# jgkellymit/GENIE-SMEM

Measured on AMD Instinct MI355X. Metric: query-bases/sec SMEM discovery, 100kb ref x 150bp reads; bit-exact SMEM set, higher is better.
Workload: dtype u8/int32 (2-bit packed bases, int32 SA rows; f64 only in the RMI predict)

## Files before the change

genie-smem_amd/csrc/kernels.hip:

```cpp
#include <hip/hip_runtime.h>

#include <algorithm>
#include <cstdio>
#include <cstdlib>
#include <mutex>
#include <string>
#include <unordered_map>

#include "genie_internal.h"

namespace genie {

namespace {

constexpr int kWave = 64;

__device__ __forceinline__ int rfl(int v) { return __builtin_amdgcn_readfirstlane(v); }
__device__ __forceinline__ void set_wave_priority(int i)
{
    switch (i & 3) {
    case 0: __builtin_amdgcn_s_setprio(0); break;
    case 1: __builtin_amdgcn_s_setprio(1); break;
    case 2: __builtin_amdgcn_s_setprio(2); break;
    default: __builtin_amdgcn_s_setprio(3); break;
// ... 455 lines not shown
__device__ __forceinline__ unsigned long long wave_inclusive_scan64(unsigned long long v, int lane)
{
#pragma unroll
    for (int off = 1; off < kWave; off <<= 1) {
        const unsigned int lo = (unsigned)__shfl_up((int)(unsigned)v, off, kWave);
        const unsigned int hi = (unsigned)__shfl_up((int)(unsigned)(v >> 32), off, kWave);
        if (lane >= off) v += ((unsigned long long)hi << 32) | lo;
    }
    return v;
}

__global__ void __launch_bounds__(kScanBlock) compact_block_sums(const int32_t *__restrict__ counts, long long N, int cap,
                                                                 unsigned long long *__restrict__ block_sums)
{
    __shared__ unsigned long long wsum[kScanBlock / kWave];
    const long long i = (long long)blockIdx.x * kScanBlock + threadIdx.x;
    unsigned long long v = 0;
    if (i < N) { const int c = counts[i]; v = (unsigned long long)(c < 0 ? 0 : (c < cap ? c : cap)); }
    v = wave_sum64(v);
    if ((threadIdx.x & 63) == 0) wsum[threadIdx.x >> 6] = v;
    __syncthreads();
    if (threadIdx.x == 0) {
        unsigned long long s = 0;
        for (int w = 0; w < kScanBlock / kWave; w++) s += wsum[w];
        block_sums[blockIdx.x] = s;
    }
}

__global__ void __launch_bounds__(kScanBlock) scan_block_sums_kernel(unsigned long long *__restrict__ sums, long long nblocks)
{
    constexpr int kPer = 8;
    __shared__ unsigned long long wave_total[kScanBlock / kWave];
    __shared__ unsigned long long carry;
    const int lane = threadIdx.x & (kWave - 1), wave = threadIdx.x >> 6;
    if (threadIdx.x == 0) carry = 0;
    __syncthreads();
    for (long long base = 0; base < nblocks; base += (long long)kScanBlock * kPer) {
        const long long i0 = base + (long long)threadIdx.x * kPer;
        unsigned long long v[kPer], mine = 0;
#pragma unroll
        for (int e = 0; e < kPer; e++) {
            v[e] = i0 + e < nblocks ? sums[i0 + e] : 0ull;
            mine += v[e];
        }
        unsigned long long inc = mine;
#pragma unroll
        for (int off = 1; off < kWave; off <<= 1) {
            const unsigned int lo = (unsigned)__shfl_up((int)(unsigned)inc, off, kWave);
            const unsigned int hi = (unsigned)__shfl_up((int)(unsigned)(inc >> 32), off, kWave);
            if (lane >= off) inc += ((unsigned long long)hi << 32) | lo;
        }
        if (lane == kWave - 1) wave_total[wave] = inc;
        __syncthreads();
        unsigned long long before = carry, all = 0;
        for (int w = 0; w < kScanBlock / kWave; w++) {
            const unsigned long long t = wave_total[w];
            before += w < wave ? t : 0ull;
            all += t;
        }
        unsigned long long run = before + inc - mine;
#pragma unroll
        for (int e = 0; e < kPer; e++) {
            if (i0 + e < nblocks) sums[i0 + e] = run;
            run += v[e];
        }
        __syncthreads();
        if (threadIdx.x == 0) carry += all;
        __syncthreads();
    }
    if (threadIdx.x == 0) sums[nblocks] = carry;
}

__global__ void __launch_bounds__(kScanBlock) compact_scatter(const int32_t *__restrict__ counts,
                                                              const int4 *__restrict__ slots, long long N, int cap,
                                                              const unsigned long long *__restrict__ block_sums,
                                                              long long *__restrict__ offsets, int4 *__restrict__ out,
                                                              long long out_cap_rows)
{
    __shared__ unsigned long long wave_total[kScanBlock / kWave];
    const int lane = threadIdx.x & (kWave - 1), wave = threadIdx.x >> 6;
    const long long i = (long long)blockIdx.x * kScanBlock + threadIdx.x;
    unsigned long long v = 0;
    if (i < N) { const int c = counts[i]; v = (unsigned long long)(c < 0 ? 0 : (c < cap ? c : cap)); }
    const unsigned long long inc = wave_inclusive_scan64(v, lane);
    if (lane == kWave - 1) wave_total[wave] = inc;
    __syncthreads();
    unsigned long long base = block_sums[blockIdx.x] + inc - v;
    for (int w = 0; w < wave; w++) base += wave_total[w];
    if (i < N) {
        offsets[i] = (long long)base;
        if (i == N - 1) offsets[N] = (long long)(base + v);
        if (out) {
            const long long room = out_cap_rows - (long long)base;
            const unsigned int fit = room <= 0 ? 0u : (room < (long long)v ? (unsigned int)room : (unsigned int)v);
            for (unsigned int t = 0; t < fit; t++) out[base + t] = slots[i * (long long)cap + t];
        }
    }
}

std::mutex g_err_mu;
std::string g_err;

#define HIP_TRY(expr)                                                         \
    do {                                                                      \
        hipError_t e_ = (expr);                                               \
        if (e_ != hipSuccess) { set_hip_error(#expr, (int)e_); return GENIE_E_HIP; } \
    } while (0)

#define LAUNCH(kernel, grid, block, lds, stream, ...)                         \
    do {                                                                      \
        hipLaunchKernelGGL(kernel, grid, block, lds, stream, __VA_ARGS__);    \
        HIP_TRY(hipGetLastError());                                           \
    } while (0)

inline long long table_bytes(const genie_index *ix)
{
    return (long long)((ix->dev.flags & kFlagCompactTable) ? sizeof(MatchRec16) : sizeof(MatchRec)) * ix->dev.mtab_entries;
}

struct Geometry {
    int grid, block, lds;
    int grp;
    int wps;
    int wide;
    int max_len;
    int fwd_stride;
    int fwd_lds;
    int qp_recs;
    int qp_stride;
    int kj_row;
};

inline void shape_for(int max_len, Geometry *g)
{
    g->max_len = max_len;
    g->wide = max_len > 255;
    g->qp_recs = g->wide ? (max_len + 31) / 32 : ((max_len + 8 + 31) / 32 + 1 + 1) / 2;
    g->fwd_stride = g->wide ? ((max_len * 2) + 15) & ~15 : std::max(16, (max_len + 15) & ~15);
    int dw = std::max(1, (max_len + 3) / 4);
    if ((dw & 1) == 0) dw++;
    g->fwd_lds = dw * 4;
    g->kj_row = (std::max(max_len, 1) + 1 + 7) & ~7;
    g->qp_stride = g->wide ? g->qp_recs : g->qp_recs + kPairHeadWords * 8 / 16;
}

int plan_find_smems(const genie_index *ix, int mode, int max_len, long long N, Geometry *g)
{
    (void)mode;
    const int lds_cap = 160 * 1024;
    shape_for(max_len, g);
    const int cus = ix->num_cus > 0 ? ix->num_cus : 256;
    const int wpb = 8;
    long long per_block;
    if (g->wide) {
        g->grp = 1;
        g->lds = wpb * mt_long_wave_bytes(max_len, g->qp_recs) + 16;
        per_block = wpb;
    } else {
        const int ml = std::max(max_len, 1);
        const int grp = ix->opt_group_positions > 0 ? ix->opt_group_positions / ml : kMtTarget / ml;
        g->grp = std::max(1, std::min(std::min(kMtMaxG, kWave / mt_pack_dwords(ml) * 4), grp));
        g->lds = wpb * mt_wave_bytes(g->grp, ml, g->qp_recs, g->fwd_stride) + 16 + mt_quad_table_bytes(g->grp, ml);
        per_block = (long long)wpb * g->grp;
    }
    if (g->lds > lds_cap) return GENIE_E_TOO_LONG;
    g->block = wpb * kWave;
    g->wps = !g->wide && table_bytes(ix) > kTableFitsL2 ? 4 : ((ix->dev.flags & kFlagCompactTable) ? 6 : 8);
    int bpc = std::min(lds_cap / g->lds, 4 * g->wps / wpb);
    if (ix->opt_search_blocks_per_cu > 0) bpc = std::min(bpc, ix->opt_search_blocks_per_cu);
    if (bpc < 1) bpc = 1;
    long long gr = (long long)cus * bpc;
    const long long need = (N + per_block - 1) / per_block;
    if (gr > need) gr = need;
    if (gr < 1) gr = 1;
    g->grid = (int)gr;
    return GENIE_OK;
}

struct Workspace {
    uint8_t *fwd;
    RefRec *qp;
    int32_t *status;
    uint8_t *kj;
    int32_t *counts;
    uint8_t *scan_tmp;
    int32_t *vlens;
};

inline int64_t ws_align(int64_t x) { return (x + 255) & ~(int64_t)255; }

struct Carver {
    uint8_t *base;
    int64_t at = 0;
    template <class T> void take(T *&piece, int64_t bytes)
    {
        piece = base ? reinterpret_cast<T *>(base + at) : nullptr;
        at += ws_align(bytes);
    }
};

template <class F>
inline long long pass_size(long long lo, long long total, F fits)
{
    long long hi = std::max(lo, total);
    while (lo < hi) {
        const long long mid = lo + (hi - lo + 1) / 2;
        if (fits(mid)) lo = mid; else hi = mid - 1;
    }
    return std::min(lo, total);
}

inline int64_t block_sums_bytes(int64_t N) { return (N / 16 + 3) * 8; }

inline int64_t workspace_layout(uint8_t *base, int64_t N, const Geometry &g, Workspace *ws, int64_t vlens_n = 0)
{
    Carver c{base};
    c.take(ws->fwd, N * (int64_t)g.fwd_stride);
    c.take(ws->qp, N * (int64_t)g.qp_stride * 16);
    c.take(ws->status, N * 4);
    c.take(ws->kj, N * (int64_t)g.kj_row * (g.wide ? 4 : 2));
    c.take(ws->counts, N * 4);
    c.take(ws->scan_tmp, block_sums_bytes(N));
    c.take(ws->vlens, vlens_n * 4);
    return c.at + 256;
}

inline int carve_workspace(void *d_ws, int64_t ws_bytes, int64_t N, const Geometry &g, Workspace *ws, int64_t vlens_n = 0)
{
    if (!d_ws || ws_bytes < workspace_layout(static_cast<uint8_t *>(d_ws), N, g, ws, vlens_n) || (reinterpret_cast<uintptr_t>(d_ws) & 255) != 0)
        return GENIE_E_CAPACITY;
    return GENIE_OK;
}

constexpr long long kLongTwoLaneReads = 32768;

struct FindRequest : FindBatch {
    int32_t *counts = nullptr, *slots = nullptr;
    int32_t cap = 0;
    int64_t *offsets = nullptr;
    int32_t *rows = nullptr;
    int64_t cap_rows = 0;
    bool packed = false;
    int row_bytes = 8;
    uint8_t *counts8 = nullptr, *status8 = nullptr;
    int64_t *escapes = nullptr;
    int64_t cap_escapes = 0;
    bool both = false;

    explicit FindRequest(const FindBatch &b) : FindBatch(b) {}
};

constexpr int kLdsBytes = 160 * 1024;
std::mutex g_lds_mu;
std::unordered_map<const void *, int> g_lds_limit;

template <class Kernel>
int allow_large_lds(Kernel k)
{
    const void *fn = reinterpret_cast<const void *>(k);
    int limit;
    {
        std::lock_guard<std::mutex> lk(g_lds_mu);
        auto it = g_lds_limit.find(fn);
        if (it == g_lds_limit.end()) {
            hipFuncAttributes attr;
            HIP_TRY(hipFuncGetAttributes(&attr, fn));
            it = g_lds_limit.emplace(fn, kLdsBytes - (int)attr.sharedSizeBytes).first;
        }
        limit = it->second;
    }
    HIP_TRY(hipFuncSetAttribute(fn, hipFuncAttributeMaxDynamicSharedMemorySize, limit));
    return GENIE_OK;
}

template <class Kernel, class... Args>
int launch_match_table(Kernel km, const Geometry &g, hipStream_t s, Args... args)
{
    if (int rc = allow_large_lds(km)) return rc;
    LAUNCH(km, dim3(g.grid), dim3(g.block), g.lds, s, args...);
    return GENIE_OK;
}

inline auto pick_interval_rows(bool c16, bool packed, int row_bytes) -> decltype(&interval_rows_kernel<true, 0>)
{
    if (!packed) return c16 ? interval_rows_kernel<true, 0> : interval_rows_kernel<false, 0>;
    if (row_bytes == 6) return c16 ? interval_rows_kernel<true, 2> : interval_rows_kernel<false, 2>;
    return c16 ? interval_rows_kernel<true, 1> : interval_rows_kernel<false, 1>;
}
inline auto pick_interval(bool csr, bool wide, bool c16) -> decltype(&interval_kernel<false, false, true>)
{
    if (csr) return c16 ? interval_kernel<true, true, true> : interval_kernel<true, true, false>;
    if (wide) return c16 ? interval_kernel<false, true, true> : interval_kernel<false, true, false>;
    return c16 ? interval_kernel<false, false, true> : interval_kernel<false, false, false>;
}

template <int MODE, bool WIDE>
int launch_pipeline(const genie_index *ix, const Geometry &g, const FindRequest &r, const Workspace &ws, hipStream_t s)
{
    int32_t *st = r.status ? r.status : ws.status;
    int32_t *cnt = r.counts ? r.counts : ws.counts;
    const bool c16 = (ix->dev.flags & kFlagCompactTable) != 0;
    const long long mtab_bytes = table_bytes(ix);
    const int cus = ix->num_cus > 0 ? ix->num_cus : 256;
    const int max_len = std::max(g.max_len, 1);
    const int long_flags = ix->opt_search_all | ix->opt_scheduling << 16, flags = long_flags | ix->opt_debug << 8;
    if (ix->ev_search_begin) HIP_TRY(hipEventRecord((hipEvent_t)ix->ev_search_begin, s));
    int rc;
    if (WIDE && r.both)
        rc = launch_match_table(c16 ? match_table_long_both_kernel<true> : match_table_long_both_kernel<false>, g, s, ix->dev,
                                (int)MODE, r.reads, r.lens, (long long)r.N, r.stride, r.fixed_len, reinterpret_cast<uint8_t *>(ws.fwd),
                                g.fwd_stride, ws.qp, g.qp_recs, st, max_len, mtab_bytes, long_flags, cus, ws.vlens);
    else if (WIDE)
        rc = launch_match_table(c16 ? match_table_long_kernel<true> : match_table_long_kernel<false>, g, s, ix->dev, (int)MODE,
                                r.reads, r.lens, (long long)r.N, r.stride, r.fixed_len, reinterpret_cast<uint8_t *>(ws.fwd),
                                g.fwd_stride, ws.qp, g.qp_recs, st, max_len, mtab_bytes, long_flags, cus);
    else if (r.both)
        rc = launch_match_table(c16 ? (g.wps == 4 ? match_table_both_kernel<4, true> : match_table_both_kernel<6, true>)
                                    : (g.wps == 4 ? match_table_both_kernel<4, false> : match_table_both_kernel<8, false>),
                                g, s, ix->dev, (int)MODE, r.reads, r.lens, (long long)r.N, r.stride, r.fixed_len,
                                reinterpret_cast<uint8_t *>(ws.fwd), g.fwd_stride, ws.qp, g.qp_recs, g.qp_stride, st, g.grp,
// ... 430 lines not shown
```

genie-smem_amd/csrc/match_table_body.inc:

```
    static_assert(!(PK && RC), "both strands of 2-bit packed reads are not built");
    typedef uint32_t __attribute__((aligned(1))) u32_unaligned;
    extern __shared__ __align__(16) uint8_t smem[];
    const int lane = threadIdx.x & (kWave - 1);
    const int wave = rfl((int)(threadIdx.x >> 6));
    const int waves_per_block = blockDim.x >> 6;
    const int dbg = (flags >> 8) & 63;
    const int sched = flags >> 16;
    const bool look_up_all = (flags & 1) != 0;
    const int FS = fwd_stride;
    const int K = ix.K;
    const int P2 = ix.P2;
    const int DW = mt_short_row_dwords(max_len, qp_recs);
    const int DWp = mt_pack_dwords(max_len);
    const int QL = mt_quads(max_len);
    const int nquads = grp * QL;
    const __amdgpu_buffer_rsrc_t mtab =
        __builtin_amdgcn_make_buffer_rsrc(const_cast<MatchRec *>(ix.mtab), 0, (int)mtab_bytes, 0x00020000);
    const __amdgpu_buffer_rsrc_t ov =
        __builtin_amdgcn_make_buffer_rsrc(const_cast<MatchOv16 *>(ix.ov), 0, ix.ov_entries * (int)sizeof(MatchOv16), 0x00020000);

    uint8_t *wb = smem + wave * mt_wave_bytes(grp, max_len, qp_recs, FS);
    uint32_t *Dp = reinterpret_cast<uint32_t *>(wb);
    int *Ls = reinterpret_cast<int *>(wb + mt_r16(grp * DW * 4));
    uint8_t *fwL = reinterpret_cast<uint8_t *>(Ls) + 64;
    uint16_t *sl = reinterpret_cast<uint16_t *>(fwL + mt_r16(grp * FS));
    uint16_t *qa = reinterpret_cast<uint16_t *>(reinterpret_cast<uint8_t *>(sl) + mt_r16(grp * max_len * 2));
    uint16_t *qb = qa + grp * mt_quads(max_len);
    for (int i = lane; i < grp * DW; i += kWave) Dp[i] = 0;
    const uint8_t *reads_end = reads + (RC ? N >> 1 : N) * (long long)stride;

    const int pu = (int)(((uint32_t)lane * (uint32_t)(65536 / DWp + 1)) >> 16);
    const int pj = lane - pu * DWp;

    uint32_t *next_group = reinterpret_cast<uint32_t *>(smem + waves_per_block * mt_wave_bytes(grp, max_len, qp_recs, FS));
    const long long groups = (N + grp - 1) / grp;
    const long long share = (groups + gridDim.x - 1) / gridDim.x;
    const long long g_begin = (long long)blockIdx.x * share;
    const long long g_end = g_begin + share < groups ? g_begin + share : groups;
    const bool handed_out = !(sched & 1), rotate = !(sched & 2);
    if (threadIdx.x == 0) *next_group = (uint32_t)waves_per_block;
    uint2 *qtab = reinterpret_cast<uint2 *>(next_group + 4);
    for (int t = threadIdx.x; t < (nquads + 191) / 192 * 192; t += blockDim.x) {
        const int tq = t < nquads ? t : 0;
        const int u = tq / QL, a = 4 * (tq - u * QL);
        const uint32_t o = 2u * (uint32_t)a + 1u;
        qtab[t] = make_uint2((uint32_t)u << 28 | (uint32_t)(u * FS + a) << 16 | (uint32_t)a,
                             ((uint32_t)(u * DW) + (o >> 5)) << 8 | (32u - (o & 31u)));
    }
    __syncthreads();
    long long gi = handed_out ? g_begin + wave : (long long)blockIdx.x * waves_per_block + wave;
    const long long g_stop = handed_out ? g_end : groups;
    const int round_of_block = (int)(blockIdx.x / (uint32_t)cus);
    const bool touch_ahead = !(sched & 8);
    for (int it = 0; gi < g_stop; it++) {
        const long long r = gi * grp;
        if (rotate) set_wave_priority(it + round_of_block);
        long long gi_next;
        if (handed_out) {
            uint32_t nx = 0;
            if (lane == 0) nx = atomicAdd(next_group, 1u);
            gi_next = g_begin + (long long)(uint32_t)rfl((int)nx);
        } else {
            gi_next = gi + (long long)gridDim.x * waves_per_block;
        }
        if (touch_ahead && stride > 0 && gi_next < g_stop) {
            const long long rn = gi_next * grp;
            const long long rows = N - rn < (long long)grp ? N - rn : (long long)grp;
            if (RC) scalar_touch_lines(reads + (rn >> 1) * (long long)stride, (uint32_t)((((rn + rows - 1) >> 1) - (rn >> 1) + 1) * stride));
            else scalar_touch_lines(reads + rn * (long long)stride, (uint32_t)(rows * stride));
        }
        bool any_read = false;
        for (int u0 = 0; u0 < grp; u0 += kWave / DWp) {
            const int u = u0 + pu;
            const bool mine = pu < kWave / DWp && u < grp;
            int L = 0, st = GENIE_READ_OK;
            uint32_t d = 0;
            bool bad = false;
            if (mine && r + u < N) {
                const long long row = RC ? (r + u) >> 1 : r + u;
                const bool rev = RC && ((r + u) & 1);
                L = lens ? lens[row] : fixed_len;
                if (RC && lens && pj == 0) vlens[r + u] = L;
                if (L < 0 || L > max_len) { st = GENIE_READ_BAD_BASE; L = 0; }
                const int left = L - 16 * pj;
                if (PK) {
                    if (left > 0) {
                        d = __builtin_bswap32(*reinterpret_cast<const uint32_t *>(reads + (r + u) * (long long)stride + 4 * pj));
                        if (left < 16) d &= ~0u << (32 - 2 * left);
                    }
                }
                const uint8_t *src = reads + row * (long long)stride + 16 * pj;
                uint32_t v[4] = {0, 0, 0, 0};
                if (PK) {
                } else if (rev) {
                    const long long o = row * (long long)stride + L - 16 - 16 * pj;
                    if (left >= 16 || (left > 0 && o >= 0)) {
                        const nt_u4 q = *reinterpret_cast<const nt_u4_unaligned *>(reads + o);
                        v[0] = __builtin_bswap32(q.w); v[1] = __builtin_bswap32(q.z); v[2] = __builtin_bswap32(q.y); v[3] = __builtin_bswap32(q.x);
                        if (left < 16) {
#pragma unroll
                            for (int k = 0; k < 4; k++) {
                                const int nb = left - 4 * k;
                                v[k] = nb >= 4 ? v[k] : (nb <= 0 ? 0u : v[k] & ((1u << (8 * nb)) - 1u));
                            }
                        }
                    } else if (left > 0) {
                        const uint8_t *f = reads + row * (long long)stride;
                        for (int b = 0; b < left; b++) v[b >> 2] |= (uint32_t)f[left - 1 - b] << (8 * (b & 3));
                    }
                } else if (left >= 16 || (left > 0 && src + 16 <= reads_end)) {
                    const nt_u4 q = *reinterpret_cast<const nt_u4_unaligned *>(src);
                    v[0] = q.x; v[1] = q.y; v[2] = q.z; v[3] = q.w;
                    if (left < 16) {
#pragma unroll
                        for (int k = 0; k < 4; k++) {
                            const int nb = left - 4 * k;
                            v[k] = nb >= 4 ? v[k] : (nb <= 0 ? 0u : v[k] & ((1u << (8 * nb)) - 1u));
                        }
                    }
                } else if (left > 0) {
#pragma unroll
                    for (int k = 0; k < 4; k++) {
                        if (left >= 4 * k + 4) v[k] = *reinterpret_cast<const u32_unaligned *>(src + 4 * k);
                        else for (int b = 0; b < left - 4 * k; b++) v[k] |= (uint32_t)src[4 * k + b] << (8 * b);
                    }
                }
                if (!PK) {
                    bad = ((v[0] | v[1] | v[2] | v[3]) & 0xFCFCFCFCu) != 0;
                    d = (mt_pack4(v[0]) << 24) | (mt_pack4(v[1]) << 16) | (mt_pack4(v[2]) << 8) | mt_pack4(v[3]);
                    if (rev && left > 0) d ^= left >= 16 ? ~0u : ~0u << (32 - 2 * left);
                }
            }
            const uint32_t prev = (uint32_t)__builtin_amdgcn_update_dpp(0, (int)d, 0x138 , 0xf, 0xf, true);
            const unsigned long long badm = __ballot(bad);
            bool ok = false;
            if (mine) {
                Dp[u * DW + pj] = __builtin_amdgcn_alignbit(prev, d, 1);
                if (pj == 0) {
                    const unsigned long long mine_bits = ((1ull << DWp) - 1ull) << (pu * DWp);
                    if (st == GENIE_READ_OK && (badm & mine_bits)) st = GENIE_READ_BAD_BASE;
                    if (st == GENIE_READ_OK && mode != GENIE_MODE_BWA && L < K) st = GENIE_READ_TOO_SHORT;
                    if (r + u < N) status[r + u] = st;
                    ok = st == GENIE_READ_OK && L > 0;
                    Ls[u] = ok ? L : 0;
                }
            }
            any_read |= __any(ok);
        }
        wave_lds_fence();
        if (any_read) {
            for (int t0 = 0; t0 < ((dbg & 8) ? 0 : grp * qp_recs); t0 += kWave) {
                const int t = t0 + lane;
                const int u = t / qp_recs, i = t - u * qp_recs;
                if (t < grp * qp_recs && Ls[u] > 0) {
                    const uint32_t *q = Dp + u * DW + 4 * i;
                    const uint32_t q0 = q[0], q1 = q[1], q2 = q[2], q3 = q[3], q4 = q[4];
                    uint4 rec;
                    rec.y = __builtin_amdgcn_alignbit(q0, q1, 31);
                    rec.x = __builtin_amdgcn_alignbit(q1, q2, 31);
                    rec.w = __builtin_amdgcn_alignbit(q2, q3, 31);
                    rec.z = __builtin_amdgcn_alignbit(q3, q4, 31);
                    store_nt(qp_out + (r + u) * (long long)qp_stride + i, rec);
                }
            }
            int nslow = 0;
#pragma nounroll
            for (int c0 = 0; c0 < ((dbg & 4) ? 0 : nquads); c0 += kMtNsp * kWave) {
                uint32_t ent[kMtNsp];
                MtProbe pr[kMtNsp];
#pragma unroll
                for (int s = 0; s < kMtNsp; s++) {
                    const int t0 = c0 + 64 * s + lane;
                    const uint2 q = qtab[t0];
                    int m = Ls[q.x >> 28] - (int)(q.x & 255u);
                    m = t0 < nquads && m > 0 ? m : 0;
                    ent[s] = q.x | ((uint32_t)m << 8);
                    const uint32_t *dq = Dp + (q.y >> 8);
                    const uint32_t sh = q.y & 255u;
                    const uint32_t d0 = dq[0], d1 = dq[1], d2 = dq[2];
                    pr[s] = mt_issue<C16>(mtab, __builtin_amdgcn_alignbit(d0, d1, sh), __builtin_amdgcn_alignbit(d1, d2, sh), P2);
                }
                mt_v4i rb[kMtNsp];
#pragma unroll
                for (int s = 0; s < kMtNsp; s++) rb[s] = mt_second<C16>(mtab, pr[s]);
#pragma unroll
                for (int s = 0; s < kMtNsp; s++) {
                    bool slow;
                    const int best0 = mt_eval<C16>(pr[s], rb[s], P2, slow);
                    const int a = (int)(ent[s] & 255u), m = (int)((ent[s] >> 8) & 255u);
                    const int best = best0 < m ? best0 : m;
                    if (m) fwL[(ent[s] >> 16) & 0xFFFu] = (uint8_t)(a + best);
                    slow = slow && m > best0;
                    const unsigned long long sb = __ballot(slow);
                    if (slow) sl[nslow + __popcll(sb & ((1ull << lane) - 1ull))] = (uint16_t)(((ent[s] >> 28) << 8) | (uint32_t)a);
                    nslow += __popcll(sb);
                }
            }
            wave_lds_fence();
#pragma nounroll
            for (int c0 = 0; c0 < ((dbg & 1) ? 0 : nslow); c0 += kWave) mt_slow<false, C16>(ix, mtab, ov, mode, lane, c0, nslow, sl, Dp, DW, Ls, fwL, FS);
            wave_lds_fence();
            nslow = 0;
            int nqa = 0, nqb = 0;
            const unsigned long long below = (1ull << lane) - 1ull;
#pragma nounroll
            for (int t0 = lane; t0 < ((dbg & 6) ? 0 : nquads) + lane; t0 += kWave) {
                const uint2 q = qtab[t0 < nquads ? t0 : 0];
                const int u = (int)(q.x >> 28), a = (int)(q.x & 255u);
                const int L = Ls[u];
                const int m = t0 < nquads && L > a ? L - a : 0;
                const uint32_t fo = (q.x >> 16) & 0xFFFu;
                const uint32_t v0 = fwL[fo];
                const bool has_right = m > 4;
                const uint32_t v4 = has_right ? fwL[fo + 4] : 0u;
                const bool need = m > 1 && (look_up_all || ((int)v0 != L && !(has_right && v4 == v0)));
                if (m && !need) *reinterpret_cast<uint32_t *>(fwL + fo) = v0 * 0x01010101u;
                const unsigned long long nb = __ballot(need);
                if (need) qa[nqa + __popcll(nb & below)] = (uint16_t)((uint32_t)u << 8 | (uint32_t)a);
                nqa += __popcll(nb);
            }
            wave_lds_fence();
#pragma nounroll
            for (int c0 = 0; c0 < nqa; c0 += kWave) {
                const bool valid = c0 + lane < nqa;
                const uint32_t it = qa[valid ? c0 + lane : 0];
                const int u = (int)(it >> 8), a = (int)(it & 255u);
                const int L = Ls[u], m = L - a;
                const int km = m > 2 ? 2 : 1;
                const uint32_t fo = __umul24((uint32_t)u, (uint32_t)FS) + (uint32_t)a;
                const uint32_t o = 2u * (uint32_t)(a + km) + 1u;
                const uint32_t *dq = Dp + __umul24((uint32_t)u, (uint32_t)DW) + (o >> 5);
                const uint32_t sh = 32u - (o & 31u);
                const uint32_t d0 = dq[0], d1 = dq[1], d2 = dq[2];
                const MtProbe pm = mt_issue<C16>(mtab, __builtin_amdgcn_alignbit(d0, d1, sh), __builtin_amdgcn_alignbit(d1, d2, sh), P2);
                const uint32_t v0 = fwL[fo];
                const bool has_right = m > 4;
                const uint32_t v4 = has_right ? fwL[fo + 4] : 0u;
                const mt_v4i rm = mt_second<C16>(mtab, pm);
                bool sm;
                const int bm = mt_eval<C16>(pm, rm, P2, sm);
                const int em = bm < m - km ? bm : m - km;
                sm = valid && sm && m - km > bm;
                const uint32_t vm = (uint32_t)(a + km + em);
                bool need1 = false, need3 = false;
                if (valid) {
                    if (km == 1) {
                        *reinterpret_cast<uint32_t *>(fwL + fo) = v0 | vm << 8;
                    } else {
                        need1 = look_up_all || sm || vm != v0;
                        need3 = m > 3 && (look_up_all || sm || !((has_right && vm == v4) || (int)vm == L));
                        *reinterpret_cast<uint32_t *>(fwL + fo) = v0 | v0 << 8 | vm << 16 | (m > 3 ? vm : 0u) << 24;
                    }
                }
                const unsigned long long sbm = __ballot(sm), b1 = __ballot(need1), b3 = __ballot(need3);
                if (sm) sl[nslow + __popcll(sbm & below)] = (uint16_t)(it + (uint32_t)km);
                nslow += __popcll(sbm);
                if (need1) qb[nqb + __popcll(b1 & below)] = (uint16_t)(it + 1u);
                nqb += __popcll(b1);
                if (need3) qb[nqb + __popcll(b3 & below)] = (uint16_t)(it + 3u);
                nqb += __popcll(b3);
            }
            wave_lds_fence();
#pragma nounroll
            for (int c0 = 0; c0 < nqb; c0 += kWave) {
                const bool valid = c0 + lane < nqb;
                const uint32_t it = qb[valid ? c0 + lane : 0];
                const int u = (int)(it >> 8), a = (int)(it & 255u);
                const int m = Ls[u] - a;
                const uint32_t o = 2u * (uint32_t)a + 1u;
                const uint32_t *dq = Dp + __umul24((uint32_t)u, (uint32_t)DW) + (o >> 5);
                const uint32_t sh = 32u - (o & 31u);
                const uint32_t d0 = dq[0], d1 = dq[1], d2 = dq[2];
                const MtProbe pn = mt_issue<C16>(mtab, __builtin_amdgcn_alignbit(d0, d1, sh), __builtin_amdgcn_alignbit(d1, d2, sh), P2);
                const mt_v4i rn = mt_second<C16>(mtab, pn);
                bool slow;
                const int b0 = mt_eval<C16>(pn, rn, P2, slow);
                const int e = b0 < m ? b0 : m;
                if (valid) fwL[__umul24((uint32_t)u, (uint32_t)FS) + (uint32_t)a] = (uint8_t)(a + e);
                slow = valid && slow && m > b0;
                const unsigned long long sb = __ballot(slow);
                if (slow) sl[nslow + __popcll(sb & below)] = (uint16_t)it;
                nslow += __popcll(sb);
            }
            wave_lds_fence();
#pragma nounroll
            for (int c0 = 0; c0 < ((dbg & 1) ? 0 : nslow); c0 += kWave) mt_slow<false, C16>(ix, mtab, ov, mode, lane, c0, nslow, sl, Dp, DW, Ls, fwL, FS);
            wave_lds_fence();
            const int nrows = N - r < (long long)grp ? (int)(N - r) : grp;
            uint4 *dst = reinterpret_cast<uint4 *>(fwd_out + r * (long long)FS);
            const uint4 *src = reinterpret_cast<const uint4 *>(fwL);
            for (int i = lane; i < ((dbg & 32) ? 0 : nrows * (FS >> 4)); i += kWave) store_nt(dst + i, src[i]);
        }
        wave_lds_fence();
        gi = gi_next;
    }
```

genie-smem_amd/csrc/match_table_kernel.inc:

```

constexpr int kMtNsp = 3;
constexpr int kMtMaxG = 16;
constexpr int kMtTarget = 768;


__host__ __device__ inline int mt_row_dwords(int max_len, int qp_recs)
{
    const int a = ((2 * (max_len + 8) + 1) >> 5) + 3, b = 2 * qp_recs + 3;
    return a > b ? a : b;
}
__host__ __device__ inline int mt_pack_dwords(int max_len) { return (max_len + 15) / 16 + 1; }
__host__ __device__ inline int mt_quads(int max_len) { return (max_len + 3) / 4; }
__host__ __device__ inline int mt_r16(int x) { return (x + 15) & ~15; }
__host__ __device__ inline int mt_quad_table_bytes(int grp, int max_len) { return (grp * mt_quads(max_len) + 191) / 192 * 192 * 8; }
__host__ __device__ inline int mt_short_row_dwords(int max_len, int chunks) { return mt_row_dwords(max_len, 2 * chunks - 1); }
__host__ __device__ inline int mt_wave_bytes(int grp, int max_len, int qp_recs, int fwd_stride)
{
    return mt_r16(grp * mt_short_row_dwords(max_len, qp_recs) * 4) + 64 + mt_r16(grp * fwd_stride) + mt_r16(grp * max_len * 2) +
           mt_r16(grp * mt_quads(max_len) * 6);
}

struct QBits {
    const uint32_t *p;
    __device__ __forceinline__ uint64_t win(int pos) const
    {
        const uint32_t o = 2u * (uint32_t)pos + 1u;
        const uint32_t *d = p + (o >> 5);
        const uint32_t s = 32u - (o & 31u);
        const uint32_t d0 = d[0], d1 = d[1], d2 = d[2];
        return ((uint64_t)__builtin_amdgcn_alignbit(d0, d1, s) << 32) | __builtin_amdgcn_alignbit(d1, d2, s);
    }
};

__device__ __forceinline__ uint32_t mt_pack4(uint32_t v) { return ((v << 6) | (v >> 4) | (v >> 14) | (v >> 24)) & 255u; }

struct MtProbe {
    uint32_t xk;
    int voff;
    mt_v4i ra;
};
template <bool C16>
__device__ __forceinline__ MtProbe mt_issue(const __amdgpu_buffer_rsrc_t mtab, uint32_t w1, uint32_t w2, int P2)
{
    MtProbe p;
    p.xk = __builtin_amdgcn_alignbit(w1, w2, 32 - 2 * P2);
    p.voff = (int)((w1 >> (32 - 2 * P2)) << (C16 ? 4 : 5));
    p.ra = __builtin_amdgcn_raw_buffer_load_b128(mtab, p.voff, 0, 0);
    return p;
}
template <bool C16>
__device__ __forceinline__ mt_v4i mt_second(const __amdgpu_buffer_rsrc_t mtab, const MtProbe &p)
{
    mt_v4i rb = mt_v4i{p.ra.z, p.ra.z, p.ra.z, p.ra.z};
    if (!C16 && ((uint32_t)p.ra.x >> 24) > 2u && p.xk > (uint32_t)p.ra.w) rb = __builtin_amdgcn_raw_buffer_load_b128(mtab, p.voff + 16, 0, 0);
    return rb;
}
typedef unsigned short mt_us2 __attribute__((ext_vector_type(2)));
__device__ __forceinline__ uint32_t mt_pk_min(uint32_t a, uint32_t b)
{
    return __builtin_bit_cast(uint32_t, __builtin_elementwise_min(__builtin_bit_cast(mt_us2, a), __builtin_bit_cast(mt_us2, b)));
}
__device__ __forceinline__ uint32_t mt_xmin16(const mt_v4i e, uint32_t xk16, bool more)
{
    const uint32_t xx = xk16 * 0x10001u;
    uint32_t d3 = (uint32_t)e.w ^ xx;
    d3 |= more ? 0xFFFF0000u : 0u;
    const uint32_t mm = mt_pk_min(mt_pk_min((uint32_t)e.y ^ xx, (uint32_t)e.z ^ xx), d3);
    return min(mm & 0xFFFFu, mm >> 16);
}
__device__ __forceinline__ int mt_lcp16(uint32_t x16) { return x16 ? (__clz((int)x16) - 16) >> 1 : 8; }
template <bool C16>
__device__ __forceinline__ int mt_eval(const MtProbe &p, const mt_v4i rb, int P2, bool &slow)
{
    if (C16) {
        const uint32_t w0 = (uint32_t)p.ra.x, cnt4 = (w0 >> 24) & 15u, nib = w0 >> 28;
        const bool wide = (nib & kM16Wide) && cnt4 >= 1u && cnt4 <= 3u;
        const bool rows_decide = cnt4 == kM16More || (cnt4 != 0 && !wide && (nib & kM16General));
        const uint32_t xx = wide ? p.xk : (p.xk >> 16) * 0x10001u;
        const uint32_t d1 = (uint32_t)p.ra.y ^ xx, d2 = (uint32_t)p.ra.z ^ xx, d3 = (uint32_t)p.ra.w ^ xx;
        const uint32_t mm = mt_pk_min(mt_pk_min(d1, d2), d3);
        const uint32_t xn = (min(mm & 0xFFFFu, mm >> 16) << 16) | 0xFFFFu;
        const uint32_t xw = min(min(d1, d2), d3);
        const int lcp = __clz((int)(wide ? xw : xn)) >> 1;
        slow = cnt4 != 0 && (rows_decide || lcp == (wide ? 16 : 8));
        return cnt4 == 0 ? (int)nib : (rows_decide ? P2 : P2 + lcp);
    }
    const uint32_t meta = (uint32_t)p.ra.x;
    uint32_t x = min(p.xk ^ (uint32_t)p.ra.z, p.xk ^ (uint32_t)p.ra.w);
    x = min(x, min(min(p.xk ^ (uint32_t)rb.x, p.xk ^ (uint32_t)rb.y), min(p.xk ^ (uint32_t)rb.z, p.xk ^ (uint32_t)rb.w)));
    const int lcp = __clz((int)x) >> 1;
    const int lm = (int)((meta >> 8) & 0x1Fu);
    slow = (meta & kMatchSlow) || lcp + lm == 16 + 0x1F;
    return (int)(meta & 0xFFu) + (lcp & lm);
}

struct MtQuad {
    uint32_t v1, v2, v3;
    bool s1, s2, s3;
};
template <bool C16>
__device__ __forceinline__ MtQuad mt_quad_interior(const __amdgpu_buffer_rsrc_t mtab, int P2, uint32_t d0, uint32_t d1, uint32_t d2,
                                                   uint32_t sh, int a, int m, int L, uint32_t v0, bool has_right, uint32_t v4,
                                                   bool look_up_all)
{
    MtQuad q{v0, 0u, 0u, false, false, false};
    const int km = m > 2 ? 2 : 1;
    const MtProbe pm = mt_issue<C16>(mtab, __builtin_amdgcn_alignbit(d0, d1, sh - 2 * km), __builtin_amdgcn_alignbit(d1, d2, sh - 2 * km), P2);
    const mt_v4i rm = mt_second<C16>(mtab, pm);
    bool sm;
    const int bm = mt_eval<C16>(pm, rm, P2, sm);
    const int em = bm < m - km ? bm : m - km;
    sm = sm && m - km > bm;
    const uint32_t vm = (uint32_t)(a + km + em);
    if (km == 1) {
        q.v1 = vm;
        q.s1 = sm;
        return q;
    }
    q.v2 = vm;
    q.s2 = sm;
    const bool need1 = look_up_all || sm || vm != v0;
    const bool need3 = m > 3 && (look_up_all || sm || !((has_right && vm == v4) || (int)vm == L));
    q.v1 = v0;
    q.v3 = m > 3 ? vm : 0u;
    if (need1 || need3) {
        const uint32_t s13 = need1 ? sh - 2 : sh - 6;
        const MtProbe pa = mt_issue<C16>(mtab, __builtin_amdgcn_alignbit(d0, d1, s13), __builtin_amdgcn_alignbit(d1, d2, s13), P2);
        MtProbe pb = pa;
        const bool both = need1 && need3;
        if (both) pb = mt_issue<C16>(mtab, __builtin_amdgcn_alignbit(d0, d1, sh - 6), __builtin_amdgcn_alignbit(d1, d2, sh - 6), P2);
        const mt_v4i ra = mt_second<C16>(mtab, pa);
        mt_v4i rb = ra;
        if (both) rb = mt_second<C16>(mtab, pb);
        bool sa, sb;
        const int ba = mt_eval<C16>(pa, ra, P2, sa), bb = mt_eval<C16>(pb, rb, P2, sb);
        const int ka = need1 ? 1 : 3;
        const int ea = ba < m - ka ? ba : m - ka, eb = bb < m - 3 ? bb : m - 3;
        sa = sa && m - ka > ba;
        sb = sb && m - 3 > bb;
        if (need1) { q.v1 = (uint32_t)(a + 1 + ea); q.s1 = sa; }
        else { q.v3 = (uint32_t)(a + 3 + ea); q.s3 = sa; }
        if (both) { q.v3 = (uint32_t)(a + 3 + eb); q.s3 = sb; }
    }
    return q;
}

template <bool LONG, bool C16, class QB = QBits, class FW = uint16_t>
__device__ __forceinline__ void mt_slow(const DevIndex &ix, const __amdgpu_buffer_rsrc_t mtab, const __amdgpu_buffer_rsrc_t ov, int mode, int lane, int c0,
                                        int count, const uint16_t *list, const uint32_t *Dp, int DW, const int *Ls,
                                        uint8_t *fwL, int FS, int L0 = 0, int wbase = 0, FW *fwW = nullptr)
{
    const int K = ix.K, P = ix.P, P2 = ix.P2;
    const int idx = c0 + lane;
    const bool on = idx < count;
    int u = 0, a = 0, m = 0, best = 0, chain = 0, cvoff = 0, nrows = 0;
    uint32_t mask = 0, lb = 0, c = 0, xmin = ~0u, xkq = 0;
    bool general = false;
    uint64_t w = 0, xq = 0;
    QB Q{reinterpret_cast<decltype(QB::p)>(Dp)};
    if (on) {
        const uint32_t e = (uint32_t)list[idx];
        if constexpr (LONG) {
            a = wbase + (int)e;
            m = L0 - a;
        } else {
            u = (int)(e >> 8);
            a = (int)(e & 255u);
            m = Ls[u] - a;
            Q.p = Dp + u * DW;
        }
        w = Q.win(a);
// ... 186 lines not shown
```

Measured before the change: 205.8 billion.

## Cap slow-path LDS list and double group size for issue-bound small tables

```diff
diff --git a/genie-smem_amd/csrc/kernels.hip b/genie-smem_amd/csrc/kernels.hip
--- a/genie-smem_amd/csrc/kernels.hip
+++ b/genie-smem_amd/csrc/kernels.hip
@@ -631,20 +631,25 @@
     const int cus = ix->num_cus > 0 ? ix->num_cus : 256;
     const int wpb = 8;
     long long per_block;
+    g->wps = !g->wide && table_bytes(ix) > kTableFitsL2 ? 4 : ((ix->dev.flags & kFlagCompactTable) ? 6 : 8);
     if (g->wide) {
         g->grp = 1;
         g->lds = wpb * mt_long_wave_bytes(max_len, g->qp_recs) + 16;
         per_block = wpb;
     } else {
         const int ml = std::max(max_len, 1);
-        const int grp = ix->opt_group_positions > 0 ? ix->opt_group_positions / ml : kMtTarget / ml;
-        g->grp = std::max(1, std::min(std::min(kMtMaxG, kWave / mt_pack_dwords(ml) * 4), grp));
-        g->lds = wpb * mt_wave_bytes(g->grp, ml, g->qp_recs, g->fwd_stride) + 16 + mt_quad_table_bytes(g->grp, ml);
+        auto group_of = [&](int positions) { return std::max(1, std::min(std::min(kMtMaxG, kWave / mt_pack_dwords(ml) * 4), positions / ml)); };
+        auto lds_of = [&](int grp) {
+            return wpb * mt_wave_bytes(grp, ml, g->qp_recs, g->fwd_stride) + 16 + mt_quad_table_bytes(grp, ml);
+        };
+        g->grp = group_of(ix->opt_group_positions > 0 ? ix->opt_group_positions : kMtTarget);
+        const bool issue_bound = g->wps != 4 && 2 * table_bytes(ix) <= kTableFitsL2;
+        if (ix->opt_group_positions <= 0 && issue_bound && lds_cap / lds_of(group_of(kMtTarget2)) >= 4 * g->wps / wpb) g->grp = group_of(kMtTarget2);
+        g->lds = lds_of(g->grp);
         per_block = (long long)wpb * g->grp;
     }
     if (g->lds > lds_cap) return GENIE_E_TOO_LONG;
     g->block = wpb * kWave;
-    g->wps = !g->wide && table_bytes(ix) > kTableFitsL2 ? 4 : ((ix->dev.flags & kFlagCompactTable) ? 6 : 8);
     int bpc = std::min(lds_cap / g->lds, 4 * g->wps / wpb);
     if (ix->opt_search_blocks_per_cu > 0) bpc = std::min(bpc, ix->opt_search_blocks_per_cu);
     if (bpc < 1) bpc = 1;
diff --git a/genie-smem_amd/csrc/match_table_body.inc b/genie-smem_amd/csrc/match_table_body.inc
--- a/genie-smem_amd/csrc/match_table_body.inc
+++ b/genie-smem_amd/csrc/match_table_body.inc
@@ -24,7 +24,7 @@
     int *Ls = reinterpret_cast<int *>(wb + mt_r16(grp * DW * 4));
     uint8_t *fwL = reinterpret_cast<uint8_t *>(Ls) + 64;
     uint16_t *sl = reinterpret_cast<uint16_t *>(fwL + mt_r16(grp * FS));
-    uint16_t *qa = reinterpret_cast<uint16_t *>(reinterpret_cast<uint8_t *>(sl) + mt_r16(grp * max_len * 2));
+    uint16_t *qa = reinterpret_cast<uint16_t *>(reinterpret_cast<uint8_t *>(sl) + mt_r16(mt_slow_cap(grp, max_len) * 2));
     uint16_t *qb = qa + grp * mt_quads(max_len);
     for (int i = lane; i < grp * DW; i += kWave) Dp[i] = 0;
     const uint8_t *reads_end = reads + (RC ? N >> 1 : N) * (long long)stride;
@@ -164,8 +164,14 @@
                 }
             }
             int nslow = 0;
-#pragma nounroll
-            for (int c0 = 0; c0 < ((dbg & 4) ? 0 : nquads); c0 += kMtNsp * kWave) {
+            int positions = grp * max_len;
+            asm volatile("" : "+s"(positions));
+            const int flush_at = positions > kMtSlowCap ? kMtSlowCap - kWave : 1 << 30;
+            const int n1 = (dbg & 4) ? 0 : nquads;
+            int c0 = 0;
+            do {
+#pragma nounroll
+            for (; c0 < n1 && nslow + (kMtNsp - 1) * kWave <= flush_at; c0 += kMtNsp * kWave) {
                 uint32_t ent[kMtNsp];
                 MtProbe pr[kMtNsp];
 #pragma unroll
@@ -198,9 +204,10 @@
             }
             wave_lds_fence();
 #pragma nounroll
-            for (int c0 = 0; c0 < ((dbg & 1) ? 0 : nslow); c0 += kWave) mt_slow<false, C16>(ix, mtab, ov, mode, lane, c0, nslow, sl, Dp, DW, Ls, fwL, FS);
+            for (int s0 = 0; s0 < ((dbg & 1) ? 0 : nslow); s0 += kWave) mt_slow<false, C16>(ix, mtab, ov, mode, lane, s0, nslow, sl, Dp, DW, Ls, fwL, FS);
             wave_lds_fence();
             nslow = 0;
+            } while (__builtin_expect(c0 < n1, 0));
             int nqa = 0, nqb = 0;
             const unsigned long long below = (1ull << lane) - 1ull;
 #pragma nounroll
@@ -220,10 +227,12 @@
                 nqa += __popcll(nb);
             }
             wave_lds_fence();
-#pragma nounroll
-            for (int c0 = 0; c0 < nqa; c0 += kWave) {
-                const bool valid = c0 + lane < nqa;
-                const uint32_t it = qa[valid ? c0 + lane : 0];
+            int cm = 0, cn = 0;
+            do {
+#pragma nounroll
+            for (; cm < nqa && nslow <= flush_at; cm += kWave) {
+                const bool valid = cm + lane < nqa;
+                const uint32_t it = qa[valid ? cm + lane : 0];
                 const int u = (int)(it >> 8), a = (int)(it & 255u);
                 const int L = Ls[u], m = L - a;
                 const int km = m > 2 ? 2 : 1;
@@ -262,9 +271,9 @@
             }
             wave_lds_fence();
 #pragma nounroll
-            for (int c0 = 0; c0 < nqb; c0 += kWave) {
-                const bool valid = c0 + lane < nqb;
-                const uint32_t it = qb[valid ? c0 + lane : 0];
+            for (; cm >= nqa && cn < nqb && nslow <= flush_at; cn += kWave) {
+                const bool valid = cn + lane < nqb;
+                const uint32_t it = qb[valid ? cn + lane : 0];
                 const int u = (int)(it >> 8), a = (int)(it & 255u);
                 const int m = Ls[u] - a;
                 const uint32_t o = 2u * (uint32_t)a + 1u;
@@ -284,8 +293,10 @@
             }
             wave_lds_fence();
 #pragma nounroll
-            for (int c0 = 0; c0 < ((dbg & 1) ? 0 : nslow); c0 += kWave) mt_slow<false, C16>(ix, mtab, ov, mode, lane, c0, nslow, sl, Dp, DW, Ls, fwL, FS);
-            wave_lds_fence();
+            for (int s0 = 0; s0 < ((dbg & 1) ? 0 : nslow); s0 += kWave) mt_slow<false, C16>(ix, mtab, ov, mode, lane, s0, nslow, sl, Dp, DW, Ls, fwL, FS);
+            wave_lds_fence();
+            nslow = 0;
+            } while (__builtin_expect(cm < nqa || cn < nqb, 0));
             const int nrows = N - r < (long long)grp ? (int)(N - r) : grp;
             uint4 *dst = reinterpret_cast<uint4 *>(fwd_out + r * (long long)FS);
             const uint4 *src = reinterpret_cast<const uint4 *>(fwL);
diff --git a/genie-smem_amd/csrc/match_table_kernel.inc b/genie-smem_amd/csrc/match_table_kernel.inc
--- a/genie-smem_amd/csrc/match_table_kernel.inc
+++ b/genie-smem_amd/csrc/match_table_kernel.inc
@@ -2,6 +2,8 @@
 constexpr int kMtNsp = 3;
 constexpr int kMtMaxG = 16;
 constexpr int kMtTarget = 768;
+constexpr int kMtTarget2 = 1536;
+constexpr int kMtSlowCap = 512;
 
 
 __host__ __device__ inline int mt_row_dwords(int max_len, int qp_recs)
@@ -14,9 +16,10 @@
 __host__ __device__ inline int mt_r16(int x) { return (x + 15) & ~15; }
 __host__ __device__ inline int mt_quad_table_bytes(int grp, int max_len) { return (grp * mt_quads(max_len) + 191) / 192 * 192 * 8; }
 __host__ __device__ inline int mt_short_row_dwords(int max_len, int chunks) { return mt_row_dwords(max_len, 2 * chunks - 1); }
+__host__ __device__ inline int mt_slow_cap(int grp, int max_len) { return grp * max_len <= kMtSlowCap ? grp * max_len : kMtSlowCap; }
 __host__ __device__ inline int mt_wave_bytes(int grp, int max_len, int qp_recs, int fwd_stride)
 {
-    return mt_r16(grp * mt_short_row_dwords(max_len, qp_recs) * 4) + 64 + mt_r16(grp * fwd_stride) + mt_r16(grp * max_len * 2) +
+    return mt_r16(grp * mt_short_row_dwords(max_len, qp_recs) * 4) + 64 + mt_r16(grp * fwd_stride) + mt_r16(mt_slow_cap(grp, max_len) * 2) +
            mt_r16(grp * mt_quads(max_len) * 6);
 }
 
```

Measured after the change: 213.8 billion, median of 6. 1.04x the previous value.
